# muellan/metacache

Hardware: AMD Instinct MI355X
Metric: Mreads/min (150 bp) (higher is better)
Workload: dtype u32

## Files before the change

### metacache_amd/csrc/gw_kernels.hip

```cpp
#include "device_common.h"

#include <algorithm>
#include <cstdlib>

namespace mcamd {

namespace {

constexpr uint32_t kGwNone = 0xFFFFFFFFu;
constexpr uint32_t kGwRounds = 128;
constexpr uint32_t kGwLoads = kGwRounds / 16;

struct __attribute__((packed, aligned(4))) U4 { uint32_t x, y, z, w; };

__device__ __forceinline__ uint32_t gw_block_shift(uint32_t maxWin)
{
    const uint32_t D = maxWin > 1 ? maxWin - 1 : 1;
    const uint32_t A = 32u - (uint32_t)__builtin_clz(64u * D - 1u);
    return A < 8u ? 8u : A;
}

template <uint32_t T1LOG2, uint32_t T2LOG2>
struct GwBloom {
    static constexpr uint32_t kW1 = (1u << T1LOG2) / 32, kW2 = (1u << T2LOG2) / 32, kWords = kW1 + kW2;
// ... 11 lines not shown
        asm("v_lshlrev_b32_e64 %0, %1, 1" : "=v"(m1) : "v"(h));
        asm("v_lshl_or_b32 %0, 1, %1, %2" : "=v"(m) : "v"(h >> 12), "v"(m1));
        return m;
    }
    __device__ __forceinline__ static uint32_t mask1_of(uint32_t h)
    {
        if constexpr (!kSame) return mask_of(h);
        uint32_t m1;
        asm("v_lshlrev_b32_e64 %0, %1, 1" : "=v"(m1) : "v"(h));
        return m1;
    }
    __device__ __forceinline__ static bool twice_hit(uint32_t word, uint32_t m) { if constexpr (kSame) return (word & m) != 0u; else return (word & m) == m; }
    __device__ __forceinline__ static bool twice_hit_h(uint32_t word, uint32_t h)
    {
        if constexpr (kSame) { uint32_t t; asm("v_bfe_u32 %0, %1, %2, 1" : "=v"(t) : "v"(word), "v"(h)); return t != 0u; }
        else { const uint32_t m = mask_of(h); return (word & m) == m; }
    }
    __device__ __forceinline__ static uint32_t seen_index(uint32_t h)
    {
        uint32_t i;
        asm("v_lshrrev_b32_e32 %0, %1, %2" : "=v"(i) : "n"(37u - T1LOG2), "v"(h));
        return i;
    }
    __device__ __forceinline__ static uint32_t twice_index(uint32_t seen, uint32_t h)
    {
        if constexpr (kSame) return seen + kW1;
        else return kW1 + ((h >> 17) & (kW2 - 1u));
    }
    __device__ __forceinline__ static void mark4(uint32_t* bits, uint32_t k0, uint32_t k1, uint32_t k2, uint32_t k3)
    {
        const uint32_t k[4] = {k0, k1, k2, k3};
        uint32_t m[4], i1[4], i2[4], old[4];
#pragma unroll
        for (int j = 0; j < 4; ++j) { const uint32_t h = hash(k[j]); m[j] = mask_of(h); i1[j] = seen_index(h); i2[j] = twice_index(i1[j], h); }
#pragma unroll
        for (int j = 0; j < 4; ++j) old[j] = atomicOr(&bits[i1[j]], m[j]);
#pragma unroll
        for (int j = 0; j < 4; ++j) if ((old[j] & m[j]) == m[j]) atomicOr(&bits[i2[j]], m[j]);
    }
    __device__ __forceinline__ static void mark(uint32_t* bits, uint32_t key)
    {
        const uint32_t h = hash(key), m = mask_of(h), i1 = seen_index(h);
        const uint32_t old = atomicOr(&bits[i1], m);
        if ((old & m) == m) atomicOr(&bits[twice_index(i1, h)], m);
    }
    __device__ __forceinline__ static bool twice(const uint32_t* bits, uint32_t key)
    {
        const uint32_t h = hash(key), m = mask1_of(h);
        return twice_hit(bits[twice_index(seen_index(h), h)], m);
    }
    __device__ __forceinline__ static bool seen(const uint32_t* bits, uint32_t key)
    {
        const uint32_t h = hash(key), m = mask_of(h);
        return (bits[seen_index(h)] & m) == m;
    }
};

struct GwFrame {
    uint32_t A, D, blockMask, inner;
    uint32_t shv, Dsh, twoDsh;
    __device__ __forceinline__ explicit GwFrame(uint32_t maxWin, bool fine = false)
    {
        A = gw_block_shift(maxWin); D = maxWin > 1 ? maxWin - 1 : 0u;
        if (fine) { A = 32u - (uint32_t)__builtin_clz((D > 1u ? D : 2u) - 1u); A = A < 8u ? 8u : A; }
        blockMask = (1u << A) - 1u; inner = (1u << A) - 2u * D;
        const uint32_t sh = 32u - A;
        asm volatile("v_mov_b32 %0, %1" : "=v"(shv) : "s"(sh));
        Dsh = D << sh; twoDsh = (2u * D) << sh;
    }
    __device__ __forceinline__ bool edge(uint32_t v) const
    {
        uint32_t t;
        asm("v_lshl_add_u32 %0, %1, %2, %3" : "=v"(t) : "v"(v), "v"(shv), "s"(Dsh));
        return t < twoDsh;
    }
};

__device__ __forceinline__ void gw_fill_rounds(uint64_t* T, uint32_t lane, uint32_t r0, uint32_t Rc, uint32_t start, uint32_t myR, uint32_t sz, uint64_t pay)
{
    for (uint32_t i = lane; i < kGwRounds; i += 64) if (r0 + i >= Rc) T[i] = 0ull;
    const uint32_t jlo = r0 > start ? r0 - start : 0u, jhi = min(myR, r0 + kGwRounds > start ? r0 + kGwRounds - start : 0u);
    for (uint32_t j = jlo; j < jhi; ++j) T[start + j - r0] = (pay + 16ull * j) | ((uint64_t)min(16u, sz - 16u * j) << 40);
}
__device__ __forceinline__ void gw_fill_rounds_scan(uint64_t* T, uint32_t* E, uint32_t lane, uint32_t Rc, uint32_t start, uint32_t myR, uint32_t sz, uint64_t pay)
{
    E[lane] = 0u; E[lane + 64u] = 0u;
    wave_lds_sync();
    if (myR && start < kGwRounds) E[start] = lane + 1u;
    wave_lds_sync();
    uint32_t lo = wave_incl_scan_max_u32(E[lane]);
    uint32_t hi = max(wave_incl_scan_max_u32(E[lane + 64u]), rdlane(lo, 63));
    const uint32_t payLo = (uint32_t)pay, payHi = (uint32_t)(pay >> 32);
#pragma unroll
    for (uint32_t h = 0; h < 2; ++h) {
        const uint32_t slot = lane + 64u * h, who = h ? hi : lo;
        const int src = (int)(who ? who - 1u : 0u);
        const uint32_t eStart = (uint32_t)__shfl((int)start, src), eSz = (uint32_t)__shfl((int)sz, src);
        const uint32_t eLo = (uint32_t)__shfl((int)payLo, src), eHi = (uint32_t)__shfl((int)payHi, src);
        const uint32_t j = slot - eStart;
        const uint64_t ep = ((uint64_t)eHi << 32) | eLo;
        T[slot] = (who && slot < Rc) ? ((ep + 16ull * j) | ((uint64_t)min(16u, eSz - 16u * j) << 40)) : 0ull;
    }
}
__device__ __forceinline__ void gw_fill_rounds_scan_at(uint64_t* T, uint32_t* E, uint32_t lane, uint32_t r0, uint32_t Rc, uint32_t start, uint32_t myR, uint32_t sz, uint64_t pay)
{
    E[lane] = 0u; E[lane + 64u] = 0u;
    wave_lds_sync();
    if (myR && start < r0 + kGwRounds && start + myR > r0) E[start > r0 ? start - r0 : 0u] = lane + 1u;
    wave_lds_sync();
    uint32_t lo = wave_incl_scan_max_u32(E[lane]);
    uint32_t hi = max(wave_incl_scan_max_u32(E[lane + 64u]), rdlane(lo, 63));
    const uint32_t payLo = (uint32_t)pay, payHi = (uint32_t)(pay >> 32);
#pragma unroll
    for (uint32_t h = 0; h < 2; ++h) {
        const uint32_t slot = lane + 64u * h, who = h ? hi : lo;
        const int src = (int)(who ? who - 1u : 0u);
        const uint32_t eStart = (uint32_t)__shfl((int)start, src), eSz = (uint32_t)__shfl((int)sz, src);
        const uint32_t eLo = (uint32_t)__shfl((int)payLo, src), eHi = (uint32_t)__shfl((int)payHi, src);
        const uint32_t j = r0 + slot - eStart;
        const uint64_t ep = ((uint64_t)eHi << 32) | eLo;
        T[slot] = (who && r0 + slot < Rc) ? ((ep + 16ull * j) | ((uint64_t)min(16u, eSz - 16u * j) << 40)) : 0ull;
    }
}
__device__ __forceinline__ void gw_load_rounds(const uint64_t* T, const uint32_t* __restrict__ values32, uint32_t grp, uint32_t sub4, uint4 (&x)[kGwLoads],
                                               uint32_t nl = kGwLoads)
{
#pragma unroll
    for (uint32_t u = 0; u < kGwLoads; ++u) {
        x[u] = make_uint4(kGwNone, kGwNone, kGwNone, kGwNone);
        if (u >= nl) continue;
        const uint64_t rd = T[u * 16 + grp];
        if (sub4 < (uint32_t)(rd >> 40)) {
            const U4 t = *reinterpret_cast<const U4*>(values32 + (rd & 0xFFFFFFFFFFull) + sub4);
            x[u] = make_uint4(t.x, t.y, t.z, t.w);
        }
    }
}
template <class Bloom>
__device__ __forceinline__ void gw_mark_rounds(uint32_t* bits, const uint4 (&x)[kGwLoads], uint32_t A, uint32_t nl = kGwLoads)
{
#pragma unroll
    for (uint32_t u = 0; u < kGwLoads; ++u)
        if (u < nl && x[u].x != kGwNone) Bloom::mark4(bits, x[u].x >> A, x[u].y >> A, x[u].z >> A, x[u].w >> A);
}
struct GwSink { uint32_t* dst; uint32_t room, n2; uint32_t* shared = nullptr; };
__device__ __forceinline__ uint32_t gw_reserve(uint32_t* shared, uint32_t tot)
{
    uint32_t at = 0;
    if (tot && __builtin_amdgcn_mbcnt_hi(~0u, __builtin_amdgcn_mbcnt_lo(~0u, 0u)) == 0u) at = atomicAdd(shared, tot);
    return (uint32_t)__builtin_amdgcn_readfirstlane((int)at);
}
template <class Bloom, bool FINE = false>
__device__ __forceinline__ void gw_take(const uint32_t* bits, const GwFrame& F, GwSink& S, uint32_t v, bool valid)
{
    const uint32_t key = v >> F.A;
    const bool keep = valid & (FINE ? (Bloom::twice(bits, key) | Bloom::seen(bits, key - 1u) | Bloom::seen(bits, key + 1u)) : (Bloom::twice(bits, key) | F.edge(v)));
    const uint64_t m = __ballot(keep);
    if (S.shared) S.n2 = gw_reserve(S.shared, (uint32_t)__popcll(m));
    if (keep) {
        const uint32_t at = __builtin_amdgcn_mbcnt_hi((uint32_t)(m >> 32), __builtin_amdgcn_mbcnt_lo((uint32_t)m, S.n2));
        if (at < S.room) S.dst[at] = v;
    }
    S.n2 += (uint32_t)__popcll(m);
}
template <class Bloom, bool CHECK, bool FINE = false>
__device__ __forceinline__ void gw_take4(const uint32_t* bits, const GwFrame& F, GwSink& S, const uint4 x, const int32_t rem)
{
    const uint32_t v[4] = {x.x, x.y, x.z, x.w};
    uint32_t m[4], wd[4];
    uint32_t mlo[FINE ? 4 : 1], wlo[FINE ? 4 : 1], mhi[FINE ? 4 : 1], whi[FINE ? 4 : 1];
#pragma unroll
    for (int j = 0; j < 4; ++j) {
        const uint32_t key = v[j] >> F.A;
        const uint32_t h = Bloom::hash(key);
        m[j] = h;
        wd[j] = bits[Bloom::twice_index(Bloom::seen_index(h), h)];
        if constexpr (FINE) {
            const uint32_t h0 = Bloom::hash(key - 1u), h1 = Bloom::hash(key + 1u);
            mlo[j] = Bloom::mask_of(h0); wlo[j] = bits[Bloom::seen_index(h0)];
            mhi[j] = Bloom::mask_of(h1); whi[j] = bits[Bloom::seen_index(h1)];
        }
    }
    uint64_t km[4]; bool kb[4];
#pragma unroll
    for (int j = 0; j < 4; ++j) {
        const bool valid = rem > j, hit = Bloom::twice_hit_h(wd[j], m[j]);
        if constexpr (FINE) {
            const bool lo = (wlo[j] & mlo[j]) == mlo[j], hi = (whi[j] & mhi[j]) == mhi[j];
            kb[j] = valid & (hit | lo | hi);
            km[j] = __ballot(valid) & (__ballot(hit) | __ballot(lo) | __ballot(hi));
        } else {
            const bool edge = F.edge(v[j]);
            kb[j] = valid & (hit | edge);
            km[j] = __ballot(valid) & (__ballot(hit) | __ballot(edge));
        }
    }
    if (S.shared) S.n2 = gw_reserve(S.shared, (uint32_t)(__popcll(km[0]) + __popcll(km[1]) + __popcll(km[2]) + __popcll(km[3])));
    uint32_t n2 = S.n2;
#pragma unroll
    for (int j = 0; j < 4; ++j) {
        if (kb[j]) {
            const uint32_t mine = __builtin_amdgcn_mbcnt_hi((uint32_t)(km[j] >> 32), __builtin_amdgcn_mbcnt_lo((uint32_t)km[j], 0u));
            uint32_t* const to = S.dst + n2;
            if (!CHECK || n2 + mine < S.room) to[mine] = v[j];
        }
        n2 += (uint32_t)__popcll(km[j]);
    }
    S.n2 = n2;
}
template <class Bloom, bool CHECK, bool FINE = false>
__device__ __forceinline__ void gw_take_rounds(const uint32_t* bits, const uint64_t* T, const GwFrame& F, GwSink& S, uint32_t grp, uint32_t sub4,
                                               const uint4 (&x)[kGwLoads], uint32_t nl = kGwLoads)
{
#pragma unroll
    for (uint32_t u = 0; u < kGwLoads; ++u) {
        if (u >= nl) continue;
        const int32_t rem = (int32_t)(uint32_t)(T[u * 16 + grp] >> 40) - (int32_t)sub4;
        gw_take4<Bloom, CHECK, FINE>(bits, F, S, x[u], rem);
    }
}

__device__ __forceinline__ uint32_t gw_pack_rems(const uint64_t* T, uint32_t grp, uint32_t sub4, uint32_t nl)
{
    uint32_t packed = 0;
#pragma unroll
    for (uint32_t u = 0; u < kGwLoads; ++u) {
        if (u >= nl) continue;
        const uint32_t cnt = (uint32_t)(T[u * 16 + grp] >> 40);
        packed |= (cnt > sub4 ? min(cnt - sub4, 4u) : 0u) << (3u * u);
    }
    return packed;
}
template <class Bloom, bool CHECK>
__device__ __forceinline__ void gw_take_rounds_packed(const uint32_t* bits, const uint32_t packed, const GwFrame& F, GwSink& S, const uint4 (&x)[kGwLoads], uint32_t nl)
{
#pragma unroll
    for (uint32_t u = 0; u < kGwLoads; ++u) if (u < nl) gw_take4<Bloom, CHECK>(bits, F, S, x[u], (int32_t)((packed >> (3u * u)) & 7u));
}

constexpr uint32_t kGwDefer = 0xFFFFFFFEu;
constexpr uint32_t kGwFallback = 0xFFFFFFFFu;

}

#ifndef MC_GW_FILTER_WPE
#define MC_GW_FILTER_WPE 4
#endif
template <uint32_t WAVES, uint32_t TLOG2, uint32_t WPE = MC_GW_FILTER_WPE>
__global__ __launch_bounds__(WAVES * 64, WPE) void gw_filter_kernel(BatchView b, DeviceTable tab, Workspace ws)
{
    using Bloom = GwBloom<TLOG2, TLOG2>;
    __shared__ uint32_t bitS[WAVES][Bloom::kWords];
    __shared__ uint64_t roundS[WAVES][kGwRounds];
    const uint32_t lane = threadIdx.x & 63u, wave = __builtin_amdgcn_readfirstlane(threadIdx.x >> 6);
    uint32_t* bits = bitS[wave];
    uint64_t* T = roundS[wave];
    const uint32_t total = ws.midCount[kCntFilter];
    const uint4* __restrict__ work = ws.midList + list_at(kListFilter, b.n);
    uint4* __restrict__ outRec = ws.midList + list_at(kListFiltered, b.n);
    const uint32_t nWaves = gridDim.x * WAVES;
    const uint32_t w0 = blockIdx.x * WAVES + wave;
    auto load_rec = [&](uint32_t w) -> uint4 { return w < total ? work[w] : make_uint4(0, 0, 0, 0); };
    const uint64_t sliceCap = ws.bigPoolCap / nWaves;
    uint32_t* const slice = reinterpret_cast<uint32_t*>(ws.bigPool) + (uint64_t)w0 * sliceCap;
    uint64_t sliceUsed = 0;
    uint32_t deferred = 0;
    uint4 rec = load_rec(w0), recNext = load_rec(w0 + nWaves);
    uint32_t esz = 0; uint64_t epay = 0;
    auto load_entries = [&](const uint4& r) {
        const uint32_t ne = (r.z >> 12) <= kGwSmallH ? min(r.z & 0xFFFu, 64u) : 0u;
        esz = lane < ne ? ws.psize[r.y + lane] : 0u;
        epay = lane < ne ? ws.ppay[r.y + lane] : 0ull;
    };
    load_entries(rec);
    const uint32_t grp = lane >> 2, sub4 = (lane & 3u) * 4u;
    for (uint32_t w = w0; w < total; w += nWaves) {
        const uint32_t q = rec.x, nent = rec.z & 0xFFFu, H = rec.z >> 12, maxWin = rec.w;
        const uint32_t sz = esz & 0xFFFFu; const uint64_t pay = epay;
        rec = recNext;
        recNext = load_rec(w + 2 * nWaves);
        load_entries(rec);
        const uint32_t myR = sz > 1 ? (sz + 15u) >> 4 : 0u;
        const uint32_t incl = wave_incl_scan_u32(myR, lane), Rc = rdlane(incl, 63);
        if (H > kGwSmallH || nent > 64u || Rc > kGwRounds || maxWin > tab.gwGap || sliceCap - sliceUsed < kGwRounds * 16u + 64u) {
            if (lane == 0) outRec[w] = make_uint4(q, 0u, kGwDefer, maxWin);
            ++deferred;
            continue;
        }
        {
            uint4* z4 = reinterpret_cast<uint4*>(bits);
#pragma unroll
            for (uint32_t i = 0; i < Bloom::kWords / 4 / 64; ++i) z4[i * 64 + lane] = make_uint4(0, 0, 0, 0);
        }
        gw_fill_rounds(T, lane, 0, Rc, incl - myR, myR, sz, pay);
        wave_lds_sync();
        const GwFrame F(maxWin);
        const uint32_t nl = (Rc + 15u) >> 4;
        uint4 x[kGwLoads];
        gw_load_rounds(T, tab.values32, grp, sub4, x, nl);
        const uint32_t sv = sz == 1 ? tab.gw_of(pay) : kGwNone;
        GwSink S{slice + sliceUsed, (uint32_t)min((uint64_t)kGwMaxKept, sliceCap - sliceUsed), 0u};
        if (sv != kGwNone) Bloom::mark(bits, sv >> F.A);
        gw_mark_rounds<Bloom>(bits, x, F.A, nl);
        wave_lds_sync();
        gw_take<Bloom>(bits, F, S, sv, sv != kGwNone);
        gw_take_rounds<Bloom, false>(bits, T, F, S, grp, sub4, x, nl);
        const bool fallback = S.n2 > S.room;
        if (lane == 0) {
            if (fallback) { ws.hitScan[q] = H; ws.qflag[q] = kFlagCands; outRec[w] = make_uint4(q, 0u, kGwFallback, maxWin); }
            else {
                outRec[w] = make_uint4(q, (uint32_t)((uint64_t)w0 * sliceCap + sliceUsed), S.n2, maxWin);
            }
        }
        if (!fallback) sliceUsed += S.n2;
        wave_lds_sync();
    }
    if (lane == 0) {
        if (ws.sliceFill) ws.sliceFill[w0] = (uint32_t)sliceUsed;
        if (deferred) atomicAdd(&ws.midCount[kCntSecond], deferred);
    }
// ... 366 lines not shown

template <bool TAX>
__device__ __forceinline__ bool gw_winners_out(const uint32_t lane, const uint32_t K, const uint32_t wv, const uint32_t wh, const uint32_t wd,
                                               const uint32_t wt, const uint32_t wlo, const uint32_t whi, mc_candidate_dev* __restrict__ out,
                                               uint32_t (&pickLo)[kLaneK], uint32_t (&pickHi)[kLaneK])
{
    bool again = false;
    if constexpr (!TAX) {
#pragma unroll
        for (uint32_t i = 0; i + 1 < kLaneK; ++i) {
            const uint32_t ti = rdlane(wt, i);
            again = again || (__ballot(lane > i && lane < K && wt == ti && ti != 0xFFFFFFFFu) != 0);
        }
    }
#pragma unroll
    for (uint32_t i = 0; i < kLaneK; ++i) { pickLo[i] = rdlane(wlo, i); pickHi[i] = rdlane(whi, i); }
    if (lane < K) {
        mc_candidate_dev e; e.tgt = wt; e.hits = wh; e.end = wv - wlo; e.beg = e.end - wd;
        if (wv == kGwNone) { e.tgt = 0xFFFFFFFFu; e.hits = 0; e.beg = 0; e.end = 0; }
        out[lane] = e;
    }
    return again;
}

}

namespace {

__device__ __forceinline__ void lk_store_entries(const Workspace& ws, const uint32_t fbase, const uint32_t nf, const uint32_t lane, const uint32_t sz, const uint64_t pay,
                                                 const uint64_t fm, const uint64_t sm, const uint32_t lincl)
{
    const uint32_t nent = (uint32_t)__popcll(fm), n1 = (uint32_t)__popcll(sm), lsz = sz > 1u ? sz : 0u;
    const uint32_t below = __builtin_amdgcn_mbcnt_hi((uint32_t)(fm >> 32), __builtin_amdgcn_mbcnt_lo((uint32_t)fm, 0u));
    const uint32_t sbelow = __builtin_amdgcn_mbcnt_hi((uint32_t)(sm >> 32), __builtin_amdgcn_mbcnt_lo((uint32_t)sm, 0u));
    if (sz != 0u) {
        const uint32_t slot = sz == 1u ? sbelow : n1 + (below - sbelow);
        const uint32_t off = sz == 1u ? slot : n1 + lincl - lsz;
        ws.psize[fbase + slot] = sz | ((off & 0xFFFu) << 16);
        ws.ppay[fbase + slot] = pay;
    } else if (lane < nf) ws.psize[fbase + nent + (lane - below)] = 0u;
}
__device__ __forceinline__ void lk_store_entries(const Workspace& ws, const uint32_t fbase, const uint32_t nf, const uint32_t lane, const uint32_t sz, const uint64_t pay)
{
    lk_store_entries(ws, fbase, nf, lane, sz, pay, __ballot(sz != 0u), __ballot(sz == 1u), wave_incl_scan_u32(sz > 1u ? sz : 0u, lane));
}
__device__ __forceinline__ void lk_load_entries(const Workspace& ws, const DeviceTable& tab, const uint32_t s, const uint32_t q, const uint32_t lane,
                                                uint32_t& fbase, uint32_t& nf, uint32_t& sz, uint64_t& pay)
{
    const uint32_t o0 = ws.winOff[q];
    fbase = o0 * s; nf = (ws.winOff[q + 1] - o0) * s;
    const uint32_t f = lane < nf ? ws.features[fbase + lane] : 0xFFFFFFFFu;
    const uint64_t e = f != 0xFFFFFFFFu ? tab.direct[f] : 0ull;
    sz = (uint32_t)e & 0xFFFFu; pay = direct_payload(e);
}

struct GwEntRecord {
    const uint4* rec;
    __device__ __forceinline__ uint2 where() const { const uint4 r6 = *rec; return make_uint2(r6.y, r6.z & 0xFFFu); }
    __device__ __forceinline__ void load(const Workspace& ws, const DeviceTable&, uint32_t, uint32_t fbase, uint32_t nent, uint32_t lane, uint32_t& sz, uint64_t& pay) const
    {
        sz = lane < nent ? (ws.psize[fbase + lane] & 0xFFFFu) : 0u;
        pay = lane < nent ? ws.ppay[fbase + lane] : 0ull;
    }
    __device__ __forceinline__ void leave(const Workspace&, const DeviceTable&, uint32_t, uint32_t) const {}
};
struct GwEntLookup {
    uint32_t fbase, nent, s;
    __device__ __forceinline__ uint2 where() const { return make_uint2(fbase, nent); }
    __device__ __forceinline__ void load(const Workspace& ws, const DeviceTable& tab, uint32_t q, uint32_t, uint32_t, uint32_t lane, uint32_t& sz, uint64_t& pay) const
    {
        uint32_t fb, nf;
        lk_load_entries(ws, tab, s, q, lane, fb, nf, sz, pay);
    }
    __device__ __forceinline__ void leave(const Workspace& ws, const DeviceTable& tab, uint32_t q, uint32_t lane) const
    {
        uint32_t fb, nf, sz; uint64_t pay;
        lk_load_entries(ws, tab, s, q, lane, fb, nf, sz, pay);
        lk_store_entries(ws, fb, nf, lane, sz, pay);
    }
};

struct GwPend {
    bool pend = false;
    uint32_t q = 0, wv = kGwNone, wh = 0, wd = 0, dir = 0, b0 = 0, b1 = 0, b2 = 0;
    __device__ __forceinline__ void bases(const DeviceTable& tab)
    {
        if (pend && wv != kGwNone) { b0 = tab.gwBase[dir]; b1 = tab.gwBase[dir + 1]; b2 = tab.gwBase[min(dir + 2, tab.gwTargets)]; }
    }
    template <bool TAX, class Ent>
    __device__ __forceinline__ void finish(const uint32_t lane, const uint32_t K, const DeviceTable& tab, const Workspace& ws, mc_candidate_dev* __restrict__ cands, const Ent& ent)
    {
        if (!pend) return;
        uint32_t t = 0xFFFFFFFFu, lo = 0, hi = 0;
        if (wv != kGwNone) {
            t = dir; lo = b0; hi = b1;
            if (wv >= b1) { ++t; lo = b1; hi = b2; }
            while (wv >= hi) { ++t; lo = hi; hi = tab.gwBase[t + 1]; }
        }
        uint32_t plo[kLaneK], phi[kLaneK];
        const bool again = gw_winners_out<TAX>(lane, K, wv, wh, wd, t, lo, hi, cands + (size_t)q * K, plo, phi);
        if (again) ent.leave(ws, tab, q, lane);
        if (lane == 0) {
            if (again) { ws.hitScan[q] = ws.qstat[q].hits; ws.qflag[q] = kFlagCands; }
            else ws.qflag[q] = kFlagDone;
        }
        pend = false;
    }
};

template <uint32_t LOG2S, bool TAX, bool DEFER, bool LONG = false, class GetV, class Ent>
__device__ __forceinline__ bool gw_count_read(const uint32_t q, const Ent& ent, const uint32_t n2, const uint32_t maxWin, GetV&& getv,
                                              uint2* slots, uint32_t* ck, uint64_t* T, const uint32_t lane, const uint32_t grp, const uint32_t sub4,
                                              const uint32_t K, const uint32_t* __restrict__ taxkey, const DeviceTable& tab, const Workspace& ws,
                                              mc_candidate_dev* __restrict__ cands, GwPend& P)
{
    constexpr uint32_t kSlots = 1u << LOG2S, kList = kSlots / 2;
    {
        uint4* k4 = reinterpret_cast<uint4*>(slots);
#pragma unroll
        for (uint32_t i = 0; i < kSlots * 8 / 16 / 64; ++i) k4[i * 64 + lane] = make_uint4(kGwNone, 0u, kGwNone, 0u);
    }
    wave_lds_sync();
    uint32_t pickLo[kLaneK], pickHi[kLaneK];
#pragma unroll
    for (uint32_t i = 0; i < kLaneK; ++i) { pickLo[i] = 0; pickHi[i] = 0; }
    uint32_t strong = 0, wv = kGwNone, wh = 0, wd = 0;
    bool again = false;
    mc_candidate_dev* out = cands + (size_t)q * K;
    if constexpr (DEFER) P.bases(tab);
    uint32_t C = 0;
    auto body = [&](auto perc) {
        constexpr uint32_t PER = decltype(perc)::value;
        uint32_t v[PER];
#pragma unroll
        for (uint32_t r = 0; r < PER; ++r) v[r] = getv(r);
        C = gw_count_numbers<LOG2S, PER, LONG ? kList : 0xFFFFFFFFu>(v, slots, ck, lane);
    };
    const uint32_t per = (n2 + 63u) / 64u;
    if constexpr (LOG2S == 9) {
        if (per <= 1) body(std::integral_constant<uint32_t, 1>{});
        else if (per <= 2) body(std::integral_constant<uint32_t, 2>{});
        else if (per <= 3) body(std::integral_constant<uint32_t, 3>{});
        else if (!LONG || per <= 4) body(std::integral_constant<uint32_t, 4>{});
        else if constexpr (LONG) {
            if (per <= 6) body(std::integral_constant<uint32_t, 6>{});
            else body(std::integral_constant<uint32_t, 8>{});
        }
    } else if constexpr (LOG2S == 10) {
        if (per <= 6) body(std::integral_constant<uint32_t, 6>{});
        else body(std::integral_constant<uint32_t, 8>{});
    } else {
        if (per <= 10) body(std::integral_constant<uint32_t, 10>{});
        else if (per <= 12) body(std::integral_constant<uint32_t, 12>{});
        else body(std::integral_constant<uint32_t, kList / 64>{});
    }
    C = __builtin_amdgcn_readfirstlane(C);
    wave_lds_sync();
    if constexpr (LONG) {
        if (C > kList) {
            if constexpr (DEFER) P.template finish<TAX>(lane, K, tab, ws, cands, ent);
            wave_lds_sync();
            return false;
        }
    }
    auto pick = [&](auto perc) {
        constexpr uint32_t PER = decltype(perc)::value;
        strong = gw_pick<LOG2S, PER, TAX>(ck, C, slots, lane, maxWin, K, taxkey, tab, wv, wh, wd);
    };
    if (C <= 64) pick(std::integral_constant<uint32_t, 1>{});
    else if (C <= 128) pick(std::integral_constant<uint32_t, 2>{});
    else if (C <= 256) pick(std::integral_constant<uint32_t, 4>{});
    else if constexpr (LOG2S >= 10) {
        if (C <= 512) pick(std::integral_constant<uint32_t, 8>{});
        else if constexpr (LOG2S >= 11) pick(std::integral_constant<uint32_t, 16>{});
    }
    strong = __builtin_amdgcn_readfirstlane(strong);
    if constexpr (DEFER) {
        P.template finish<TAX>(lane, K, tab, ws, cands, ent);
        if (strong >= K) {
            P.pend = true; P.q = q; P.wv = wv; P.wh = wh; P.wd = wd;
            P.dir = wv != kGwNone ? tab.gwDir[wv >> tab.gwDirShift] : 0u;
            wave_lds_sync();
            return true;
        }
    }
    {
        uint32_t wt = 0xFFFFFFFFu, wlo = 0, whi = 0;
        if (wv != kGwNone) tab.gw_target_bounds(wv, wt, wlo, whi);
        again = gw_winners_out<TAX>(lane, K, wv, wh, wd, wt, wlo, whi, out, pickLo, pickHi);
    }
    bool done = true;
    if (again) {
        ent.leave(ws, tab, q, lane);
        if (lane == 0) { ws.hitScan[q] = ws.qstat[q].hits; ws.qflag[q] = kFlagCands; }
        done = false;
    } else if (strong < K) {
        const uint2 r6 = ent.where();
        const uint32_t fbase = r6.x, nent = r6.y;
        if (TAX || nent > kBigEnt) {
            ent.leave(ws, tab, q, lane);
            if (lane == 0) { ws.hitScan[q] = ws.qstat[q].hits; ws.qflag[q] = kFlagCands; }
            done = false;
        } else if constexpr (!TAX) {
            wave_lds_sync();
            uint32_t sz; uint64_t pay;
            ent.load(ws, tab, q, fbase, nent, lane, sz, pay);
            const uint32_t myR = sz > 1 ? (sz + 15u) >> 4 : 0u;
            const uint32_t incl = wave_incl_scan_u32(myR, lane), Rc = rdlane(incl, 63), start = incl - myR;
            uint32_t best[kLaneK];
#pragma unroll
            for (uint32_t i = 0; i < kLaneK; ++i) best[i] = kGwNone;
            uint32_t seen = 0;
            auto visit = [&](uint32_t g, bool valid) {
                if (!valid) return;
                bool skip = false;
#pragma unroll
                for (uint32_t i = 0; i < kLaneK; ++i) skip = skip || (i < strong && g - pickLo[i] < pickHi[i] - pickLo[i]);
                if (skip) return;
                ++seen;
                uint32_t c = g;
#pragma unroll
                for (uint32_t i = 0; i < kLaneK; ++i) { const uint32_t lo = min(best[i], c); c = max(best[i], c); best[i] = lo; }
            };
            visit(sz == 1 ? tab.gw_of(pay) : kGwNone, sz == 1);
            for (uint32_t r0 = 0; r0 < Rc; r0 += kGwRounds) {
                for (uint32_t i = lane; i < kGwRounds; i += 64) if (r0 + i >= Rc) T[i] = 0ull;
                const uint32_t jlo = r0 > start ? r0 - start : 0u, jhi = min(myR, r0 + kGwRounds > start ? r0 + kGwRounds - start : 0u);
                for (uint32_t j = jlo; j < jhi; ++j) T[start + j - r0] = (pay + 16ull * j) | ((uint64_t)min(16u, sz - 16u * j) << 40);
                wave_lds_sync();
#pragma unroll
                for (uint32_t u = 0; u < kGwLoads; ++u) {
                    const uint64_t rd = T[u * 16 + grp];
                    const int32_t rem = (int32_t)(uint32_t)(rd >> 40) - (int32_t)sub4;
                    if (rem > 0) {
                        const U4 t = *reinterpret_cast<const U4*>(tab.values32 + (rd & 0xFFFFFFFFFFull) + sub4);
                        visit(t.x, true); visit(t.y, rem > 1); visit(t.z, rem > 2); visit(t.w, rem > 3);
                    }
                }
                wave_lds_sync();
            }
            const bool dropped = seen > kLaneK;
            bool unsure = false;
            for (uint32_t rnd = strong; rnd < K; ++rnd) {
                if (__ballot(dropped && best[0] == kGwNone)) { unsure = true; break; }
                const uint32_t m = wave_min_u32(best[0]);
                mc_candidate_dev e; e.tgt = 0xFFFFFFFFu; e.hits = 0; e.beg = 0; e.end = 0;
                if (m != kGwNone) {
                    const uint32_t t = tab.gw_target(m), lo = tab.gwBase[t], hi = tab.gwBase[t + 1];
                    e.tgt = t; e.hits = 1; e.beg = e.end = m - lo;
                    uint32_t kept[kLaneK];
#pragma unroll
                    for (uint32_t i = 0; i < kLaneK; ++i) kept[i] = kGwNone;
                    uint32_t n = 0;
#pragma unroll
                    for (uint32_t i = 0; i < kLaneK; ++i) {
                        const bool stay = best[i] != kGwNone && !(best[i] - lo < hi - lo);
#pragma unroll
                        for (uint32_t j = 0; j < kLaneK; ++j) if (stay && j == n) kept[j] = best[i];
                        n += stay ? 1u : 0u;
                    }
#pragma unroll
                    for (uint32_t i = 0; i < kLaneK; ++i) best[i] = kept[i];
                }
// ... 6 lines not shown
            }
        }
    }
    if (done && lane == 0) ws.qflag[q] = kFlagDone;
    wave_lds_sync();
    return true;
}

}

#ifndef MC_GW_COUNT_WPE
#define MC_GW_COUNT_WPE 6
#endif
template <uint32_t LOG2S, uint32_t WAVES, bool TAX>
__global__ __launch_bounds__(WAVES * 64, LOG2S == 9 ? MC_GW_COUNT_WPE : LOG2S == 10 ? 5 : 1) void gw_count_kernel(BatchView b, uint32_t s, DeviceTable tab, Workspace ws, uint32_t K,
                                                                                             const uint32_t* __restrict__ taxkey, mc_candidate_dev* __restrict__ cands,
                                                                                             uint32_t minN2)
{
    constexpr uint32_t kSlots = 1u << LOG2S, kList = kSlots / 2;
    static_assert(kGwRounds * 8 <= kSlots * 8, "step D's round table lives in the slot table, which is done with by then");
    __shared__ __attribute__((aligned(16))) uint2 slotS[WAVES][kSlots];
    __shared__ uint32_t ckS[WAVES][kList];
    const uint32_t lane = threadIdx.x & 63u, wave = __builtin_amdgcn_readfirstlane(threadIdx.x >> 6);
    uint2* slots = slotS[wave];
    uint32_t* ck = ckS[wave];
    uint64_t* T = reinterpret_cast<uint64_t*>(slotS[wave]);
    const uint32_t total = ws.midCount[kCntFilter];
    const uint4* __restrict__ work = ws.midList + list_at(kListFiltered, b.n);
    const uint4* __restrict__ work6 = ws.midList + list_at(kListFilter, b.n);
    const uint32_t nWaves = gridDim.x * WAVES;
    const uint32_t w0 = blockIdx.x * WAVES + wave;
    const uint32_t grp = lane >> 2, sub4 = (lane & 3u) * 4u;
    const uint32_t* __restrict__ pool = reinterpret_cast<const uint32_t*>(ws.bigPool);
    constexpr uint32_t kPre = LOG2S <= 10 ? kList / 64 : 1;
    uint32_t pre[kPre];
    auto fetch = [&](uint32_t off, uint32_t n) {
        if constexpr (LOG2S <= 10) {
#pragma unroll
            for (uint32_t r = 0; r < kPre; ++r) pre[r] = r * 64 + lane < n ? pool[off + r * 64 + lane] : kGwNone;
        }
    };
    constexpr bool kDefer = LOG2S <= 10;
    GwPend P;
    const uint32_t nmine = LOG2S == 9 ? total : ws.midCount[LOG2S == 10 ? kCnt512 : kCnt1024];
    const uint32_t kStep = LOG2S == 9 ? 64u : min(8u, max(1u, (nmine + nWaves - 1) / nWaves));
    const uint32_t* __restrict__ side = ws.sideList + list_at(LOG2S == 10 ? kSide512 : kSide1024, b.n);
    for (uint32_t chunk = w0 * kStep; chunk < nmine; chunk += nWaves * kStep) {
      const bool inb = lane < kStep && chunk + lane < nmine;
      const uint32_t myW = LOG2S == 9 ? chunk + lane : (inb ? side[chunk + lane] : 0u);
      const uint4 myRec = inb ? work[myW] : make_uint4(0, 0, kGwFallback, 0);
      uint64_t todo = __ballot(myRec.z <= kList && (minN2 == 0 || myRec.z > minN2) && myRec.w <= kHashWin);
      if (todo) { const uint32_t j = (uint32_t)__ffsll((unsigned long long)todo) - 1; fetch(rdlane(myRec.y, j), rdlane(myRec.z, j)); }
      while (todo) {
        const uint32_t j = (uint32_t)__ffsll((unsigned long long)todo) - 1;
        todo &= todo - 1;
        const uint32_t w = rdlane(myW, j), q = rdlane(myRec.x, j), n2 = rdlane(myRec.z, j), maxWin = rdlane(myRec.w, j);
        const uint32_t* __restrict__ src = pool + rdlane(myRec.y, j);
        uint32_t cur[kPre];
#pragma unroll
        for (uint32_t r = 0; r < kPre; ++r) cur[r] = pre[r];
        if (todo) { const uint32_t jn = (uint32_t)__ffsll((unsigned long long)todo) - 1; fetch(rdlane(myRec.y, jn), rdlane(myRec.z, jn)); }
        gw_count_read<LOG2S, TAX, kDefer>(q, GwEntRecord{work6 + w}, n2, maxWin, [&](uint32_t r) -> uint32_t {
            if constexpr (LOG2S <= 10) return cur[r < kPre ? r : 0];
            else return r * 64 + lane < n2 ? src[r * 64 + lane] : kGwNone;
        }, slots, ck, T, lane, grp, sub4, K, taxkey, tab, ws, cands, P);
      }
    }
    if constexpr (kDefer) { P.bases(tab); P.template finish<TAX>(lane, K, tab, ws, cands, GwEntRecord{work6}); }
}

constexpr uint32_t kGwCounted = 0x80000000u;

template <uint32_t WAVES, uint32_t TLOG2, bool TAX, uint32_t WPE = MC_GW_FILTER_WPE, bool LOOKUP = false>
__global__ __launch_bounds__(WAVES * 64, WPE) void gw_filter_count_kernel(BatchView b, DeviceTable tab, Workspace ws, uint32_t K, const uint32_t* __restrict__ taxkey,
                                                                                 mc_candidate_dev* __restrict__ cands, const uint32_t s)
{
    using Bloom = GwBloom<TLOG2, TLOG2>;
    constexpr uint32_t kKeep = WPE >= 6 ? 384 : 512;
    static_assert(kGwRounds * 8 >= 256 * 4, "the distinct numbers' slots take the place of the round table");
    constexpr bool kSeven = WPE >= 7;
    __shared__ __attribute__((aligned(16))) uint32_t bitS[WAVES][Bloom::kWords];
    __shared__ __attribute__((aligned(16))) uint64_t roundS[kSeven ? 1 : WAVES][kSeven ? 1 : kGwRounds];
    __shared__ __attribute__((aligned(16))) uint32_t keptS[WAVES][kKeep];
    const uint32_t lane = threadIdx.x & 63u, wave = __builtin_amdgcn_readfirstlane(threadIdx.x >> 6);
    uint32_t* bits = bitS[wave];
    uint64_t* T = kSeven ? reinterpret_cast<uint64_t*>(bits) : roundS[kSeven ? 0 : wave];
    uint32_t* kept = keptS[wave];
    const uint32_t total = LOOKUP ? b.n : ws.midCount[kCntFilter];
    uint4* const work = ws.midList + list_at(kListFilter, b.n);
    uint4* __restrict__ outRec = ws.midList + list_at(kListFiltered, b.n);
    const uint32_t nWaves = gridDim.x * WAVES;
    const uint32_t w0 = blockIdx.x * WAVES + wave;
    auto load_rec = [&](uint32_t w) -> uint4 { return (!LOOKUP && w < total) ? work[w] : make_uint4(0, 0, 0, 0); };
    const uint64_t sliceCap = ws.bigPoolCap / nWaves;
    uint32_t* const slice = reinterpret_cast<uint32_t*>(ws.bigPool) + (uint64_t)w0 * sliceCap;
    uint64_t sliceUsed = (LOOKUP && ws.sliceFill) ? ws.sliceFill[w0] : 0u;
    uint32_t deferred = 0;
    uint4 rec = load_rec(w0), recNext = load_rec(w0 + nWaves);
    uint32_t esz = 0; uint64_t epay = 0;
    auto load_entries = [&](const uint4& r) {
        if constexpr (LOOKUP) return;
        const uint32_t ne = (r.z >> 12) <= kGwSmallH ? min(r.z & 0xFFFu, 64u) : 0u;
        esz = lane < ne ? ws.psize[r.y + lane] : 0u;
        epay = lane < ne ? ws.ppay[r.y + lane] : 0ull;
    };
    load_entries(rec);
    constexpr uint32_t kLkSkip = 0xFFFFFFFFu;
    auto load_meta = [&](uint32_t q) -> uint2 {
        if (!LOOKUP || q >= b.n) return make_uint2(kLkSkip, 0u);
        const uint32_t o0 = ws.winOff[q], nf = (ws.winOff[q + 1] - o0) * s;
        return (ws.qflag[q] == kFlagProbe && nf <= 64u) ? make_uint2(o0 * s, nf) : make_uint2(kLkSkip, 0u);
    };
    auto load_feat = [&](const uint2& m) -> uint32_t { return (m.x != kLkSkip && lane < m.y) ? ws.features[m.x + lane] : 0xFFFFFFFFu; };
    uint2 m0 = load_meta(w0), m1 = load_meta(w0 + nWaves), m2 = load_meta(w0 + 2 * nWaves);
    uint32_t lkFeat = 0xFFFFFFFFu, lkNfeat = 0; uint64_t lkEnt = 0;
    if constexpr (LOOKUP) {
        const uint32_t f0 = load_feat(m0);
        lkFeat = load_feat(m1);
        lkNfeat = (uint32_t)__popcll(__ballot(f0 != 0xFFFFFFFFu));
        lkEnt = f0 != 0xFFFFFFFFu ? tab.direct[f0] : 0ull;
    }
    const uint32_t grp = lane >> 2, sub4 = (lane & 3u) * 4u;
    GwPend P;
    for (uint32_t w = w0; w < total; w += nWaves) {
        uint32_t q, nent, H, maxWin, sz, fbase = 0, nfs = 0; uint64_t pay;
        uint32_t rix = 0xFFFFFFFFu;
        if constexpr (!LOOKUP) {
            q = rec.x; nent = rec.z & 0xFFFu; H = rec.z >> 12; maxWin = rec.w;
            sz = esz & 0xFFFFu; pay = epay;
            rec = recNext;
            recNext = load_rec(w + 2 * nWaves);
            load_entries(rec);
        } else {
            const uint2 cur = m0; const uint64_t e = lkEnt; const uint32_t nfeat = lkNfeat;
            lkNfeat = (uint32_t)__popcll(__ballot(lkFeat != 0xFFFFFFFFu));
            lkEnt = lkFeat != 0xFFFFFFFFu ? tab.direct[lkFeat] : 0ull;
            lkFeat = load_feat(m2);
            m0 = m1; m1 = m2; m2 = load_meta(w + 3 * nWaves);
            if (cur.x == kLkSkip) continue;
            q = w; fbase = cur.x; nfs = cur.y;
            sz = (uint32_t)e & 0xFFFFu; pay = direct_payload(e);
            const uint64_t fm = __ballot(sz != 0u), sm = __ballot(sz == 1u);
            nent = (uint32_t)__popcll(fm);
            const uint32_t n1 = (uint32_t)__popcll(sm), lsz = sz > 1u ? sz : 0u;
            const uint32_t lincl = wave_incl_scan_u32(lsz, lane);
            H = n1 + rdlane(lincl, 63);
            maxWin = b.maxWin ? b.maxWin[q] : b.maxWinUniform;
            if (lane == 0) { QueryStat qs; qs.hits = H; qs.nfeat = nfeat; qs.nfound = nent; qs.nsteps = nfeat; ws.qstat[q] = qs; }
            if (H == 0) {
                if (lane < K) { mc_candidate_dev ev; ev.tgt = 0xFFFFFFFFu; ev.hits = 0; ev.beg = 0; ev.end = 0; cands[(size_t)q * K + lane] = ev; }
                if (lane == 0) { ws.hitScan[q] = 0u; ws.qflag[q] = kFlagDone; }
                continue;
            }
            const bool hashOK = nent <= kHashEnt && maxWin <= kHashWin;
            const bool bigOK = H > ws.bigMin && H > 64u && nent <= 0xFFFu && maxWin <= tab.gwGap && H <= kMaxHitsPerQuery;
            const uint32_t cls = bigOK ? kClassFilter : H <= 64 ? kListMid64 : H <= 128 ? (hashOK ? kListHash256 : kListMid128) : H <= kMidMax ? (hashOK ? kListHash256 : kListMid256)
                               : (H <= kHashMax && hashOK) ? (H <= kHashMax / 2 ? kListHash512 : kListHash1024) : kClassWave;
            if (lane == 0) {
                ws.hitScan[q] = (H <= kMaxHitsPerQuery && H > kLdsCap && !(cls >= kListHash512 && cls != kClassWave)) ? H : 0u;
                ws.qflag[q] = cls != kClassWave ? kFlagMid : kFlagCands;
                if (cls != kClassWave && cls != kClassFilter) {
                    const uint32_t at = atomicAdd(&ws.midCount[class_counter(cls)], 1u);
                    ws.midList[list_at(class_list(cls), b.n) + at] = make_uint4(q, fbase, nent | (H << 12), maxWin);
                }
            }
            if (cls != kClassFilter) { lk_store_entries(ws, fbase, nfs, lane, sz, pay, fm, sm, lincl); continue; }
        }
        auto entries_out = [&]() { if constexpr (LOOKUP) GwEntLookup{fbase, nent, s}.leave(ws, tab, q, lane); };
        auto slot_of = [&]() -> uint32_t {
            if constexpr (!LOOKUP) return w;
            else {
                if (rix == 0xFFFFFFFFu) {
                    uint32_t at = 0;
                    if (lane == 0) { at = atomicAdd(&ws.midCount[kCntFilter], 1u); work[at] = make_uint4(q, fbase, nent | (H << 12), maxWin); }
                    rix = rdlane(at, 0);
                }
                return rix;
            }
        };
        const uint32_t myR = sz > 1 ? (sz + 15u) >> 4 : 0u;
        const uint32_t incl = wave_incl_scan_u32(myR, lane), Rc = rdlane(incl, 63);
        if (H > kGwSmallH || nent > 64u || Rc > kGwRounds || maxWin > tab.gwGap || sliceCap - sliceUsed < kGwRounds * 16u + 64u) {
            if constexpr (LOOKUP) lk_store_entries(ws, fbase, nfs, lane, sz, pay);
            const uint32_t at = slot_of();
            if (lane == 0) outRec[at] = make_uint4(q, 0u, kGwDefer, maxWin);
            ++deferred;
            continue;
        }
        auto clear_bits = [&]() {
            uint4* z4 = reinterpret_cast<uint4*>(bits);
#pragma unroll
            for (uint32_t i = 0; i < Bloom::kWords / 4 / 64; ++i) z4[i * 64 + lane] = make_uint4(0, 0, 0, 0);
        };
        if constexpr (!kSeven) clear_bits();
        gw_fill_rounds_scan(T, kept, lane, Rc, incl - myR, myR, sz, pay);
        wave_lds_sync();
        const GwFrame F(maxWin);
        const uint32_t nl = (Rc + 15u) >> 4;
        uint4 x[kGwLoads];
        gw_load_rounds(T, tab.values32, grp, sub4, x, nl);
        uint32_t rems = 0;
        if constexpr (kSeven) {
            rems = gw_pack_rems(T, grp, sub4, nl);
            wave_lds_sync();
            clear_bits();
            wave_lds_sync();
        }
        auto take_rounds = [&](auto check, GwSink& S) {
            constexpr bool CHECK = decltype(check)::value;
            if constexpr (kSeven) gw_take_rounds_packed<Bloom, CHECK>(bits, rems, F, S, x, nl);
            else gw_take_rounds<Bloom, CHECK>(bits, T, F, S, grp, sub4, x, nl);
        };
        const uint32_t sv = sz == 1 ? tab.gw_of(pay) : kGwNone;
        if (sv != kGwNone) Bloom::mark(bits, sv >> F.A);
        gw_mark_rounds<Bloom>(bits, x, F.A, nl);
        wave_lds_sync();
        const bool here = maxWin <= kHashWin;
        uint32_t n2;
        if (here) {
            GwSink S{kept, kKeep, 0u};
            gw_take<Bloom>(bits, F, S, sv, sv != kGwNone);
            take_rounds(std::true_type{}, S);
            n2 = S.n2;
        } else {
            GwSink S{slice + sliceUsed, (uint32_t)min((uint64_t)kGwMaxKept, sliceCap - sliceUsed), 0u};
            gw_take<Bloom>(bits, F, S, sv, sv != kGwNone);
            take_rounds(std::false_type{}, S);
            n2 = S.n2;
        }
        if (here && n2 <= kKeep) {
            if constexpr (!LOOKUP) { if (lane == 0) outRec[w] = make_uint4(q, 0u, kGwCounted | n2, maxWin); }
            wave_lds_sync();
            auto count = [&](const auto& ent) {
                return gw_count_read<9, TAX, true, true>(q, ent, n2, maxWin,
                                        [&](uint32_t r) -> uint32_t { return r * 64 + lane < n2 ? kept[r * 64 + lane] : kGwNone; },
                                        reinterpret_cast<uint2*>(bits), kSeven ? kept : reinterpret_cast<uint32_t*>(T), kSeven ? reinterpret_cast<uint64_t*>(kept) : T,
                                        lane, grp, sub4, K, taxkey, tab, ws, cands, P);
            };
            bool counted;
            if constexpr (LOOKUP) counted = count(GwEntLookup{fbase, nent, s});
            else counted = count(GwEntRecord{work + w});
            if (!counted && kSeven) {
                entries_out();
                const uint32_t at = slot_of();
                if (lane == 0) outRec[at] = make_uint4(q, 0u, kGwDefer, maxWin);
                ++deferred;
                wave_lds_sync();
            } else if (!counted) {
#pragma unroll
                for (uint32_t r = 0; r < kKeep / 64; ++r) if (r * 64 + lane < n2) slice[sliceUsed + r * 64 + lane] = kept[r * 64 + lane];
                entries_out();
                const uint32_t at = slot_of();
                if (lane == 0) outRec[at] = make_uint4(q, (uint32_t)((uint64_t)w0 * sliceCap + sliceUsed), n2, maxWin);
                sliceUsed += n2;
                wave_lds_sync();
            }
            continue;
        }
        if (here) {
            GwSink S{slice + sliceUsed, (uint32_t)min((uint64_t)kGwMaxKept, sliceCap - sliceUsed), 0u};
            gw_take<Bloom>(bits, F, S, sv, sv != kGwNone);
            take_rounds(std::false_type{}, S);
            n2 = S.n2;
        }
        const uint32_t room = (uint32_t)min((uint64_t)kGwMaxKept, sliceCap - sliceUsed);
        const bool fallback = n2 > room;
        entries_out();
        const uint32_t at = slot_of();
        if (lane == 0) {
            if (fallback) { ws.hitScan[q] = H; ws.qflag[q] = kFlagCands; outRec[at] = make_uint4(q, 0u, kGwFallback, maxWin); }
            else outRec[at] = make_uint4(q, (uint32_t)((uint64_t)w0 * sliceCap + sliceUsed), n2, maxWin);
        }
        if (!fallback) sliceUsed += n2;
        wave_lds_sync();
    }
    P.bases(tab);
    if constexpr (LOOKUP) P.template finish<TAX>(lane, K, tab, ws, cands, GwEntLookup{0u, 0u, s});
    else P.template finish<TAX>(lane, K, tab, ws, cands, GwEntRecord{work});
    if (lane == 0) {
        if (ws.sliceFill) ws.sliceFill[w0] = (uint32_t)sliceUsed;
        if (deferred) atomicAdd(&ws.midCount[kCntSecond], deferred);
    }
}

constexpr uint32_t kGwBigSorted = 8192;

template <bool TAX>
__device__ __forceinline__ void gw_sorted_scan(const uint32_t* __restrict__ g, const uint32_t first, const uint32_t end, const uint32_t D,
                                               const DeviceTable& tab, const uint32_t* __restrict__ taxkey, const uint32_t K, uint32_t* ring,
                                               const uint32_t lane, LaneCand (&top)[kLaneK], uint32_t (&toptax)[kLaneK])
{
    uint32_t cT = 0xFFFFFFFFu, cHits = 0, cBeg = 0, cEnd = 0, cLo = 0, cHi = 0;
    uint32_t lowFst = 0;
    uint32_t gnext = first + lane < end ? g[first + lane] : 0xFFFFFFFFu;
    uint32_t dnext = gnext != 0xFFFFFFFFu ? tab.gwDir[gnext >> tab.gwDirShift] : 0u;
    for (uint32_t base = first; base < end; base += 64) {
        const uint32_t cnt = min(64u, end - base), ei = base + lane;
        const bool valid = lane < cnt;
        const uint32_t gi = gnext, di = dnext;
        gnext = ei + 64u < end ? g[ei + 64u] : 0xFFFFFFFFu;
        ring[ei & 127u] = gi;
        wave_lds_sync();
        const uint32_t want = gi - D;
        const uint32_t rlo = base >= first + 64u ? base - 64u : first;
        uint32_t lo = 0, hi = 0;
        bool glob = false;
        if (valid) {
            if (lowFst >= rlo) { lo = lowFst; hi = ei; }
            else if (ring[rlo & 127u] < want) { lo = rlo + 1u; hi = ei; }
            else { lo = lowFst; hi = rlo; glob = true; }
        }
        while (__ballot(!glob && lo < hi)) {
            const uint32_t mid = (lo + hi) >> 1;
            if (!glob && lo < hi) { if (ring[mid & 127u] < want) lo = mid + 1u; else hi = mid; }
        }
        while (__ballot(glob && lo < hi)) {
            const uint32_t mid = (lo + hi) >> 1;
            if (glob && lo < hi) { if (g[mid] < want) lo = mid + 1u; else hi = mid; }
        }
        const uint32_t fst = lo;
        const uint32_t gf = !valid ? 0u : fst >= rlo ? ring[fst & 127u] : g[fst];
        lowFst = rdlane(fst, cnt - 1u);
        uint32_t t = 0xFFFFFFFFu, tlo = 0, thi = 0;
        const bool inCur = cT != 0xFFFFFFFFu && (gi - cLo) < (cHi - cLo);
        if (valid) {
            if (inCur) { t = cT; tlo = cLo; thi = cHi; }
            else {
                t = di;
                const uint32_t b0 = tab.gwBase[t], b1 = tab.gwBase[t + 1], b2 = tab.gwBase[min(t + 2, tab.gwTargets)];
                tlo = b0; thi = b1;
                if (gi >= b1) { ++t; tlo = b1; thi = b2; }
                while (gi >= thi) { ++t; tlo = thi; thi = tab.gwBase[t + 1]; }
            }
        }
        if (cT != 0xFFFFFFFFu && rdlane(t, 0) != cT && lane == 0) {
            LaneCand c; c.tgt = cT; c.hits = cHits; c.beg = cBeg; c.end = cEnd;
            top_insert(top, toptax, c, K, TAX ? taxkey : nullptr, 0xFFFFFFFFu);
        }
        uint32_t val = valid ? (((ei - fst + 1u) << 6) | (63u - lane)) : 0u;
#pragma unroll
        for (uint32_t d = 1; d < 64; d <<= 1) {
            const uint32_t ov = (uint32_t)__shfl_up((int)val, d), ot = (uint32_t)__shfl_up((int)t, d);
            if (lane >= d && ot == t) val = max(val, ov);
        }
        const uint32_t tnext = (uint32_t)__shfl_down((int)t, 1);
        const bool tail = valid && (lane + 1u >= cnt || tnext != t);
        const uint32_t wl = 63u - (val & 63u);
        LaneCand c; c.tgt = t; c.hits = val >> 6;
        c.beg = (uint32_t)__shfl((int)gf, (int)wl) - tlo; c.end = (uint32_t)__shfl((int)gi, (int)wl) - tlo;
        if (t == cT && cHits >= c.hits) { c.hits = cHits; c.beg = cBeg; c.end = cEnd; }
        const bool last = base + 64u >= end;
        if (tail && (last || lane + 1u < cnt)) top_insert(top, toptax, c, K, TAX ? taxkey : nullptr, 0xFFFFFFFFu);
        cT = rdlane(c.tgt, cnt - 1u); cHits = rdlane(c.hits, cnt - 1u); cBeg = rdlane(c.beg, cnt - 1u); cEnd = rdlane(c.end, cnt - 1u);
        cLo = rdlane(tlo, cnt - 1u); cHi = rdlane(thi, cnt - 1u);
        dnext = gnext != 0xFFFFFFFFu ? tab.gwDir[gnext >> tab.gwDirShift] : 0u;
    }
    wave_lds_sync();
// ... 183 lines not shown
```

Baseline: 20950.

## Restructure lookup prefetch pipeline and trim lane shuffles in gather-window kernel

Replaces __shfl with direct ds_bpermute and changes the lookup-mode prefetch. Per-query metadata (winOff pair and qflag) now comes in as one lane-parallel load that is decoded with readlane. The next feature load is deferred until after the take phase so it overlaps counting. Several loops gain an early break for the lookup path, the singleton payload base lookup is hoisted ahead of the round loads, and GwPend packs two fields into one register. An empty asm barrier on the lane value is added to steer register allocation. All of this aims to cut latency and register pressure, but it adds control-flow complexity and risks changing scheduling unpredictably.

```diff
diff --git a/metacache_amd/csrc/gw_kernels.hip b/metacache_amd/csrc/gw_kernels.hip
--- a/metacache_amd/csrc/gw_kernels.hip
+++ b/metacache_amd/csrc/gw_kernels.hip
@@ -117,6 +117,7 @@
     const uint32_t jlo = r0 > start ? r0 - start : 0u, jhi = min(myR, r0 + kGwRounds > start ? r0 + kGwRounds - start : 0u);
     for (uint32_t j = jlo; j < jhi; ++j) T[start + j - r0] = (pay + 16ull * j) | ((uint64_t)min(16u, sz - 16u * j) << 40);
 }
+__device__ __forceinline__ uint32_t gw_lane_value(uint32_t v, int src) { return (uint32_t)__builtin_amdgcn_ds_bpermute(src << 2, (int)v); }
 __device__ __forceinline__ void gw_fill_rounds_scan(uint64_t* T, uint32_t* E, uint32_t lane, uint32_t Rc, uint32_t start, uint32_t myR, uint32_t sz, uint64_t pay)
 {
     E[lane] = 0u; E[lane + 64u] = 0u;
@@ -130,8 +131,8 @@
     for (uint32_t h = 0; h < 2; ++h) {
         const uint32_t slot = lane + 64u * h, who = h ? hi : lo;
         const int src = (int)(who ? who - 1u : 0u);
-        const uint32_t eStart = (uint32_t)__shfl((int)start, src), eSz = (uint32_t)__shfl((int)sz, src);
-        const uint32_t eLo = (uint32_t)__shfl((int)payLo, src), eHi = (uint32_t)__shfl((int)payHi, src);
+        const uint32_t eStart = gw_lane_value(start, src), eSz = gw_lane_value(sz, src);
+        const uint32_t eLo = gw_lane_value(payLo, src), eHi = gw_lane_value(payHi, src);
         const uint32_t j = slot - eStart;
         const uint64_t ep = ((uint64_t)eHi << 32) | eLo;
         T[slot] = (who && slot < Rc) ? ((ep + 16ull * j) | ((uint64_t)min(16u, eSz - 16u * j) << 40)) : 0ull;
@@ -150,8 +151,8 @@
     for (uint32_t h = 0; h < 2; ++h) {
         const uint32_t slot = lane + 64u * h, who = h ? hi : lo;
         const int src = (int)(who ? who - 1u : 0u);
-        const uint32_t eStart = (uint32_t)__shfl((int)start, src), eSz = (uint32_t)__shfl((int)sz, src);
-        const uint32_t eLo = (uint32_t)__shfl((int)payLo, src), eHi = (uint32_t)__shfl((int)payHi, src);
+        const uint32_t eStart = gw_lane_value(start, src), eSz = gw_lane_value(sz, src);
+        const uint32_t eLo = gw_lane_value(payLo, src), eHi = gw_lane_value(payHi, src);
         const uint32_t j = r0 + slot - eStart;
         const uint64_t ep = ((uint64_t)eHi << 32) | eLo;
         T[slot] = (who && r0 + slot < Rc) ? ((ep + 16ull * j) | ((uint64_t)min(16u, eSz - 16u * j) << 40)) : 0ull;
@@ -171,12 +172,14 @@
         }
     }
 }
-template <class Bloom>
+template <class Bloom, bool LEAVE = false>
 __device__ __forceinline__ void gw_mark_rounds(uint32_t* bits, const uint4 (&x)[kGwLoads], uint32_t A, uint32_t nl = kGwLoads)
 {
 #pragma unroll
-    for (uint32_t u = 0; u < kGwLoads; ++u)
-        if (u < nl && x[u].x != kGwNone) Bloom::mark4(bits, x[u].x >> A, x[u].y >> A, x[u].z >> A, x[u].w >> A);
+    for (uint32_t u = 0; u < kGwLoads; ++u) {
+        if (u >= nl) { if constexpr (LEAVE) break; else continue; }
+        if (x[u].x != kGwNone) Bloom::mark4(bits, x[u].x >> A, x[u].y >> A, x[u].z >> A, x[u].w >> A);
+    }
 }
 struct GwSink { uint32_t* dst; uint32_t room, n2; uint32_t* shared = nullptr; };
 __device__ __forceinline__ uint32_t gw_reserve(uint32_t* shared, uint32_t tot)
@@ -255,22 +258,26 @@
     }
 }
 
+template <bool LEAVE = false>
 __device__ __forceinline__ uint32_t gw_pack_rems(const uint64_t* T, uint32_t grp, uint32_t sub4, uint32_t nl)
 {
     uint32_t packed = 0;
 #pragma unroll
     for (uint32_t u = 0; u < kGwLoads; ++u) {
-        if (u >= nl) continue;
+        if (u >= nl) { if constexpr (LEAVE) break; else continue; }
         const uint32_t cnt = (uint32_t)(T[u * 16 + grp] >> 40);
         packed |= (cnt > sub4 ? min(cnt - sub4, 4u) : 0u) << (3u * u);
     }
     return packed;
 }
-template <class Bloom, bool CHECK>
+template <class Bloom, bool CHECK, bool LEAVE = false>
 __device__ __forceinline__ void gw_take_rounds_packed(const uint32_t* bits, const uint32_t packed, const GwFrame& F, GwSink& S, const uint4 (&x)[kGwLoads], uint32_t nl)
 {
 #pragma unroll
-    for (uint32_t u = 0; u < kGwLoads; ++u) if (u < nl) gw_take4<Bloom, CHECK>(bits, F, S, x[u], (int32_t)((packed >> (3u * u)) & 7u));
+    for (uint32_t u = 0; u < kGwLoads; ++u) {
+        if (u >= nl) { if constexpr (LEAVE) break; else continue; }
+        gw_take4<Bloom, CHECK>(bits, F, S, x[u], (int32_t)((packed >> (3u * u)) & 7u));
+    }
 }
 
 constexpr uint32_t kGwDefer = 0xFFFFFFFEu;
@@ -803,9 +810,10 @@
 
 struct GwPend {
     bool pend = false;
-    uint32_t q = 0, wv = kGwNone, wh = 0, wd = 0, dir = 0, b0 = 0, b1 = 0, b2 = 0;
+    uint32_t q = 0, wv = kGwNone, whd = 0, dir = 0, b0 = 0, b1 = 0, b2 = 0;
     __device__ __forceinline__ void bases(const DeviceTable& tab)
     {
+        b0 = b1 = b2 = 0u;
         if (pend && wv != kGwNone) { b0 = tab.gwBase[dir]; b1 = tab.gwBase[dir + 1]; b2 = tab.gwBase[min(dir + 2, tab.gwTargets)]; }
     }
     template <bool TAX, class Ent>
@@ -819,7 +827,7 @@
             while (wv >= hi) { ++t; lo = hi; hi = tab.gwBase[t + 1]; }
         }
         uint32_t plo[kLaneK], phi[kLaneK];
-        const bool again = gw_winners_out<TAX>(lane, K, wv, wh, wd, t, lo, hi, cands + (size_t)q * K, plo, phi);
+        const bool again = gw_winners_out<TAX>(lane, K, wv, whd & 0xFFFFu, whd >> 16, t, lo, hi, cands + (size_t)q * K, plo, phi);
         if (again) ent.leave(ws, tab, q, lane);
         if (lane == 0) {
             if (again) { ws.hitScan[q] = ws.qstat[q].hits; ws.qflag[q] = kFlagCands; }
@@ -899,7 +907,7 @@
     if constexpr (DEFER) {
         P.template finish<TAX>(lane, K, tab, ws, cands, ent);
         if (strong >= K) {
-            P.pend = true; P.q = q; P.wv = wv; P.wh = wh; P.wd = wd;
+            P.pend = true; P.q = q; P.wv = wv; P.whd = wh | (wd << 16);
             P.dir = wv != kGwNone ? tab.gwDir[wv >> tab.gwDirShift] : 0u;
             wave_lds_sync();
             return true;
@@ -1072,7 +1080,8 @@
     __shared__ __attribute__((aligned(16))) uint32_t bitS[WAVES][Bloom::kWords];
     __shared__ __attribute__((aligned(16))) uint64_t roundS[kSeven ? 1 : WAVES][kSeven ? 1 : kGwRounds];
     __shared__ __attribute__((aligned(16))) uint32_t keptS[WAVES][kKeep];
-    const uint32_t lane = threadIdx.x & 63u, wave = __builtin_amdgcn_readfirstlane(threadIdx.x >> 6);
+    uint32_t lane = threadIdx.x & 63u;
+    const uint32_t wave = __builtin_amdgcn_readfirstlane(threadIdx.x >> 6);
     uint32_t* bits = bitS[wave];
     uint64_t* T = kSeven ? reinterpret_cast<uint64_t*>(bits) : roundS[kSeven ? 0 : wave];
     uint32_t* kept = keptS[wave];
@@ -1096,23 +1105,37 @@
     };
     load_entries(rec);
     constexpr uint32_t kLkSkip = 0xFFFFFFFFu;
-    auto load_meta = [&](uint32_t q) -> uint2 {
-        if (!LOOKUP || q >= b.n) return make_uint2(kLkSkip, 0u);
-        const uint32_t o0 = ws.winOff[q], nf = (ws.winOff[q + 1] - o0) * s;
-        return (ws.qflag[q] == kFlagProbe && nf <= 64u) ? make_uint2(o0 * s, nf) : make_uint2(kLkSkip, 0u);
+    auto load_raw = [&](uint32_t q) -> uint32_t {
+        uint32_t raw = 0u;
+        if (LOOKUP && q < b.n && lane < 3u) raw = *(lane < 2u ? ws.winOff + q + lane : ws.qflag + q);
+        return raw;
+    };
+    auto decode_raw = [&](uint32_t raw) -> uint2 {
+        const uint32_t o0 = rdlane(raw, 0), nf = (rdlane(raw, 1) - o0) * s;
+        return (LOOKUP && rdlane(raw, 2) == kFlagProbe && nf <= 64u) ? make_uint2(o0 * s, nf) : make_uint2(kLkSkip, 0u);
     };
     auto load_feat = [&](const uint2& m) -> uint32_t { return (m.x != kLkSkip && lane < m.y) ? ws.features[m.x + lane] : 0xFFFFFFFFu; };
-    uint2 m0 = load_meta(w0), m1 = load_meta(w0 + nWaves), m2 = load_meta(w0 + 2 * nWaves);
-    uint32_t lkFeat = 0xFFFFFFFFu, lkNfeat = 0; uint64_t lkEnt = 0;
+    uint2 mA = make_uint2(kLkSkip, 0u), mB = mA;
+    uint32_t lkFeat = 0xFFFFFFFFu, lkNfeat = 0, lkRaw = 0; uint64_t lkEnt = 0;
     if constexpr (LOOKUP) {
-        const uint32_t f0 = load_feat(m0);
-        lkFeat = load_feat(m1);
+        mA = decode_raw(load_raw(w0)); mB = decode_raw(load_raw(w0 + nWaves));
+        const uint32_t f0 = load_feat(mA);
+        lkFeat = load_feat(mB);
+        lkRaw = load_raw(w0 + 2 * nWaves);
         lkNfeat = (uint32_t)__popcll(__ballot(f0 != 0xFFFFFFFFu));
         lkEnt = f0 != 0xFFFFFFFFu ? tab.direct[f0] : 0ull;
     }
-    const uint32_t grp = lane >> 2, sub4 = (lane & 3u) * 4u;
+    uint32_t grp = lane >> 2, sub4 = (lane & 3u) * 4u;
+    auto hide_lane = [&]() {
+        if constexpr (LOOKUP) { asm volatile("" : "+v"(lane)); grp = lane >> 2; sub4 = (lane & 3u) * 4u; }
+    };
     GwPend P;
     for (uint32_t w = w0; w < total; w += nWaves) {
+      bool advanced = false;
+      auto advance = [&]() {
+          if constexpr (LOOKUP) { lkFeat = load_feat(mB); lkRaw = load_raw(w + 3 * nWaves); advanced = true; }
+      };
+      do {
         uint32_t q, nent, H, maxWin, sz, fbase = 0, nfs = 0; uint64_t pay;
         uint32_t rix = 0xFFFFFFFFu;
         if constexpr (!LOOKUP) {
@@ -1122,11 +1145,12 @@
             recNext = load_rec(w + 2 * nWaves);
             load_entries(rec);
         } else {
-            const uint2 cur = m0; const uint64_t e = lkEnt; const uint32_t nfeat = lkNfeat;
+            hide_lane();
+            const uint2 cur = mA; const uint64_t e = lkEnt; const uint32_t nfeat = lkNfeat;
+            const uint2 mC = decode_raw(lkRaw);
             lkNfeat = (uint32_t)__popcll(__ballot(lkFeat != 0xFFFFFFFFu));
             lkEnt = lkFeat != 0xFFFFFFFFu ? tab.direct[lkFeat] : 0ull;
-            lkFeat = load_feat(m2);
-            m0 = m1; m1 = m2; m2 = load_meta(w + 3 * nWaves);
+            mA = mB; mB = mC;
             if (cur.x == kLkSkip) continue;
             q = w; fbase = cur.x; nfs = cur.y;
             sz = (uint32_t)e & 0xFFFFu; pay = direct_payload(e);
@@ -1187,23 +1211,27 @@
         wave_lds_sync();
         const GwFrame F(maxWin);
         const uint32_t nl = (Rc + 15u) >> 4;
+        const uint32_t svLow = sz == 1 ? (uint32_t)pay : 0u;
+        const uint32_t svBase = sz == 1 ? tab.gwBase[(uint32_t)(pay >> 32)] : kGwNone;
         uint4 x[kGwLoads];
         gw_load_rounds(T, tab.values32, grp, sub4, x, nl);
+        const uint32_t sv = svBase + svLow;
         uint32_t rems = 0;
         if constexpr (kSeven) {
-            rems = gw_pack_rems(T, grp, sub4, nl);
+            rems = gw_pack_rems<LOOKUP>(T, grp, sub4, nl);
+            hide_lane();
             wave_lds_sync();
             clear_bits();
             wave_lds_sync();
         }
         auto take_rounds = [&](auto check, GwSink& S) {
             constexpr bool CHECK = decltype(check)::value;
-            if constexpr (kSeven) gw_take_rounds_packed<Bloom, CHECK>(bits, rems, F, S, x, nl);
+            if constexpr (kSeven) gw_take_rounds_packed<Bloom, CHECK, LOOKUP>(bits, rems, F, S, x, nl);
             else gw_take_rounds<Bloom, CHECK>(bits, T, F, S, grp, sub4, x, nl);
         };
-        const uint32_t sv = sz == 1 ? tab.gw_of(pay) : kGwNone;
         if (sv != kGwNone) Bloom::mark(bits, sv >> F.A);
-        gw_mark_rounds<Bloom>(bits, x, F.A, nl);
+        gw_mark_rounds<Bloom, LOOKUP>(bits, x, F.A, nl);
+        hide_lane();
         wave_lds_sync();
         const bool here = maxWin <= kHashWin;
         uint32_t n2;
@@ -1219,6 +1247,8 @@
             n2 = S.n2;
         }
         if (here && n2 <= kKeep) {
+            hide_lane();
+            advance();
             if constexpr (!LOOKUP) { if (lane == 0) outRec[w] = make_uint4(q, 0u, kGwCounted | n2, maxWin); }
             wave_lds_sync();
             auto count = [&](const auto& ent) {
@@ -1263,6 +1293,8 @@
         }
         if (!fallback) sliceUsed += n2;
         wave_lds_sync();
+      } while (false);
+      if (!advanced) advance();
     }
     P.bases(tab);
     if constexpr (LOOKUP) P.template finish<TAX>(lane, K, tab, ws, cands, GwEntLookup{0u, 0u, s});
```

Measured after the change: 23130, median of 6. 10.4% higher.
